# furcelay/gigalens

Hardware: AMD Instinct MI355X
Metric: forward+grad lens sims/sec, 128x128 px batch 1024; achieved HBM GB/s vs peak (higher is better)
Workload: dtype f32; 1 GPU; C2: EPL+shear lens, Sersic source, 128x128 px, batch 1024 per GPU, fp32 (BASELINE.json configs[1]); samples_per_gpu=1024, pixels=16384, z_dim=13, mode=fwdgrad, parallelism=single GPU

## Files before the change

### gigalens_amd/csrc/gigalens_hip.hip

```cpp
#include <algorithm>
#include <cmath>
#include <memory>
#include <cstdarg>
#include <cstdio>
#include <cstdlib>
#include <cstring>
#include <new>
#include <vector>

#include "gl_host_tables.h"
#include "gl_host.hip.h"
#include "gl_static.hip.h"
#include "gl_post.hip.h"
#include "gl_frontend.hip.h"
#include "gl_finalize.hip.h"

using namespace glk;

static thread_local char g_err[512] = "";

namespace glk {
int fail(int code, const char* fmt, ...) {
  va_list ap;
  va_start(ap, fmt);
  vsnprintf(g_err, sizeof(g_err), fmt, ap);
  va_end(ap);
  return code;
}
}

namespace {

int env_int(const char* name, int dflt) {
  const char* s = getenv(name);
  return (s && *s) ? atoi(s) : dflt;
}

void chunking(const gl_model* m, int B, int* chunk, int* n_chunks) {
  const long long tile_px = (long long)WG * 4;
  long long want = std::max<long long>((768 + B - 1) / B, ((long long)m->N + 8191) / 8192);
  if (m->target_wgs_set || !m->static_id) want = std::max<long long>(1, (m->target_wgs + B - 1) / B);
  long long per = ((long long)m->N + want - 1) / want;
  per = std::max(tile_px, (per + tile_px - 1) / tile_px * tile_px);
  if (m->chunk_px_override > 0) per = m->chunk_px_override;
  *chunk = (int)per;
  *n_chunks = (int)(((long long)m->N + per - 1) / per);
}

bool wave_front_end(const gl_model* m) { return m->has_epl && (int)m->comps.size() <= 64 && m->wave_prep; }
bool order_in_front_end(const gl_model* m, int B) {
  return wave_front_end(m) && m->use_order && m->order_fused && m->epl_comp >= 0 && B >= 2;
}

int tail_plan(const gl_model* m, int B, int n_chunks, int* tail_from, int* n_rows) {
  *tail_from = B;
  *n_rows = n_chunks;
  const bool pair_epl = m->pair && (m->static_id == ST_EPLSHEAR_SERSIC || m->static_id == ST_EPLSHEAR_SERSIC_SERSIC);
  if (m->tail_rows == 0 || !pair_epl || m->has_post || !order_in_front_end(m, B) || B > 1024) return 0;
  const int tiles = (m->N + 2 * WG - 1) / (2 * WG);
  const int slots = 256 * (m->static_id == ST_EPLSHEAR_SERSIC ? 3 : 2);
  int n_tail = m->tail_n, rows = m->tail_rows;
  if (n_tail < 0) {
    const long long wgs = (long long)B * n_chunks, rem = wgs % slots;
    if (wgs < slots || rem * 4 < slots) return 0;
    n_tail = (int)(rem / n_chunks);
  }
  if (rows < 0) rows = 2 * n_chunks;
  if (n_tail <= 0 || n_tail > B || rows > tiles || rows == n_chunks) return 0;
  *tail_from = B - n_tail;
  *n_rows = std::max(n_chunks, rows);
  return rows;
}

PostArgs post_args(const gl_model* m, float scale) {
  PostArgs p{};
  p.keff = m->d_psf;
  p.KH = m->KH; p.KW = m->KW; p.pt = m->pad_t; p.pl = m->pad_l;
  p.Hs = m->height; p.Ws = m->width; p.ss = m->supersample;
  p.H = m->height / m->supersample; p.W = m->width / m->supersample;
  p.scale = scale;
  return p;
}
constexpr bool corr_reachable(int kwp, int ncj, int ox) { return !(ox == 16 && kwp > 28) && !(ncj == 2 && kwp > 20); }
template <int KWP, int ST, int KS, int NCJ, int OX>
bool corr_launch(dim3 grid, size_t sh, hipStream_t stream, const float* in, float* out, const CorrArgs& a, std::atomic<const void*>* last) {
  if constexpr (corr_reachable(KWP, NCJ, OX)) {
    auto* fn = gl_corr_pair_kernel<KWP, ST, KS, NCJ, OX>;
    if (sh > 64 * 1024) {
      static const hipError_t big = hipFuncSetAttribute(reinterpret_cast<const void*>(fn), hipFuncAttributeMaxDynamicSharedMemorySize, 80 * 1024);
      if (big != hipSuccess) return false;
    }
    hipLaunchKernelGGL(fn, grid, dim3(CORR_GT * KS), sh, stream, in, out, a);
    if (last) last->store(reinterpret_cast<const void*>(fn), std::memory_order_relaxed);
    return true;
  } else {
    return false;
  }
}
bool launch_corr(const gl_model::CorrPlan& pl, int B, const float* in, float* out, float scale, hipStream_t stream, int dbg = 0,
                 int max_pairs_env = 0, int corr_wide = 1, std::atomic<const void*>* last = nullptr) {
  if (!pl.ok) return false;
  CorrArgs a = pl.args;
  a.B = B;
  a.scale = scale;
  a.dbg = dbg;
  a.vec = (a.Wi % 4 == 0 && a.Wout % 4 == 0 && ((reinterpret_cast<uintptr_t>(in) | reinterpret_cast<uintptr_t>(out)) & 15) == 0) ? 1 : 0;
  const bool wide = pl.ST == 2 && a.ncj == 1 && pl.KWP <= 28 && pl.max_KH <= 28 && corr_wide;
  const int ox = wide ? 16 : CORR_OX, ks = wide ? 8 : pl.ST == 2 ? 4 : 2;
  const int TR = (CORR_TR - 1) * pl.ST + pl.max_KH, TC = corr_tile_width((CORR_TCG * ox - 1) * pl.ST + pl.KWP) | 1;
  const size_t sh = std::max((size_t)TR * TC * sizeof(float2), (size_t)(ks - 1) * a.ncj * ox * CORR_GT * sizeof(float2) +
                                                                   (size_t)2 * CORR_TR * CORR_TCG * ox * a.ncj * sizeof(float));
  if (sh > (wide ? 80 : 64) * 1024) return false;
  const int max_pairs = max_pairs_env > 0 ? max_pairs_env : 65535 / a.n_class;
  if ((B + 1) / 2 > max_pairs) {
    for (int b_lo = 0; b_lo < B; b_lo += 2 * max_pairs) {
      const int nb = std::min(B - b_lo, 2 * max_pairs);
      if (!launch_corr(pl, nb, in + (size_t)b_lo * a.Hi * a.Wi, out + (size_t)b_lo * a.Hout * a.Wout, scale, stream, dbg, max_pairs_env, corr_wide, last)) return false;
    }
    return true;
  }
  const dim3 grid((pl.max_Wo + CORR_TCG * ox - 1) / (CORR_TCG * ox), (pl.max_Ho + CORR_TR - 1) / CORR_TR,
                  (unsigned)(a.n_class * ((B + 1) / 2)));
#define GL_CORR(KWP_, ST_, KS_, NCJ_, OX_) return corr_launch<KWP_, ST_, KS_, NCJ_, OX_>(grid, sh, stream, in, out, a, last);
#define GL_CORR_W(ST_, KS_, NCJ_, OX_)                                                                                          \
  switch (pl.KWP) {                                                                                                             \
    case 4: GL_CORR(4, ST_, KS_, NCJ_, OX_) case 8: GL_CORR(8, ST_, KS_, NCJ_, OX_) case 12: GL_CORR(12, ST_, KS_, NCJ_, OX_)     \
    case 16: GL_CORR(16, ST_, KS_, NCJ_, OX_) case 20: GL_CORR(20, ST_, KS_, NCJ_, OX_) case 24: GL_CORR(24, ST_, KS_, NCJ_, OX_) \
    case 28: GL_CORR(28, ST_, KS_, NCJ_, OX_) case 32: GL_CORR(32, ST_, KS_, NCJ_, OX_)                                          \
    default: return false;                                                                                                      \
  }
  if (wide) { GL_CORR_W(2, 8, 1, 16) }
  if (pl.ST == 2 && a.ncj == 1) { GL_CORR_W(2, 4, 1, CORR_OX) }
  if (pl.ST == 1 && a.ncj == 1) { GL_CORR_W(1, 2, 1, CORR_OX) }
  if (pl.ST == 1 && a.ncj == 2) { GL_CORR_W(1, 2, 2, CORR_OX) }
#undef GL_CORR_W
#undef GL_CORR
  return false;
}

}

namespace glk {

LaunchPlan launch_plan(const gl_model* m, int B) {
  LaunchPlan p{};
  chunking(m, B, &p.chunk, &p.n_chunks);
  p.tail_rows = tail_plan(m, B, p.n_chunks, &p.tail_from, &p.n_rows);
  return p;
}

Workspace carve(const gl_model* m, int B, void* base, const LaunchPlan& plan) {
  Workspace w{};
  size_t off = 0;
  char* p = (char*)base;
  w.derived = (float*)(p + off);
  off += align_up((size_t)B * m->D * sizeof(float), 256);
  w.partial = (float*)(p + off);
  off += align_up((size_t)B * plan.n_rows * m->A * sizeof(float), 256);
  w.params = (float*)(p + off);
  off += align_up((size_t)B * std::max(m->P, 1) * sizeof(float), 256);
  w.order = (int*)(p + off);
  off += align_up((size_t)B * sizeof(int), 256);
  w.cost = (int*)(p + off);
  off += align_up((size_t)B * sizeof(int), 256);
  if (m->G) {
    w.gal_dyn = (float*)(p + off);
    off += align_up((size_t)B * m->G * GM_ND * sizeof(float), 256);
  }
  if (m->pos_J) {
    auto take = [&](size_t n) { float* q = (float*)(p + off); off += align_up(n * sizeof(float), 256); return q; };
    w.pos_w = take((size_t)B * m->pos_J * 6);
    w.pos_adj = take((size_t)B * m->pos_J * 3);
    w.pos_g = take((size_t)B * m->pos_J * std::max(m->P, 1));
    w.pos_fam = take((size_t)B * m->pos_F * 2);
    w.pos_ll = take(B);
    w.pos_chi2 = take(B);
    w.pos_grad = take((size_t)B * std::max(m->P, 1));
    w.pos_dadj = take((size_t)B * m->pos_J);
  }
  if (m->has_post) {
    w.img_ss = (float*)(p + off);
    off += align_up((size_t)B * m->height * m->width * sizeof(float), 256);
    w.img_tmp = (float*)(p + off);
    off += align_up((size_t)B * (m->height / m->supersample) * (m->width / m->supersample) * sizeof(float), 256);
    w.stats = (float*)(p + off);
    off += align_up((size_t)B * 2 * sizeof(float), 256);
  } else if (m->mp_K >= 2) {
    w.img_tmp = (float*)(p + off);
    off += align_up((size_t)B * m->height * m->width * sizeof(float), 256);
    w.stats = (float*)(p + off);
    off += align_up((size_t)B * 2 * sizeof(float), 256);
  }
  w.bytes = off;
  return w;
}

MainArgs base_args(const gl_model* m, const Workspace& w, int chunk) {
  MainArgs a{};
  a.comps = m->d_comps;
  a.n_lens = m->n_lens;
  a.n_ll = m->n_ll;
  a.n_src = m->n_src;
  a.derived = w.derived;
  a.D = m->D;
  a.A = m->A;
  a.Apad = m->Apad;
  a.ncols = m->ncols;
  a.gx = m->d_gx;
  a.gy = m->d_gy;
  a.pix = m->d_pix;
  a.N = m->N;
  a.chunk = chunk;
  a.img_stride = (long long)m->height * m->width;
  a.out_scale = m->conversion_factor;
  a.partial = w.partial;
  a.shp_tab = m->d_shp_tab;
  a.nfw_tab = m->d_nfw_tab;
  a.neutral = m->d_nfw_tab ? m->d_nfw_tab + 2 * glh::kNfwNodes : nullptr;
  a.grid_rmax = m->shp_cull ? m->grid_rmax : -1.f;
  a.dbg = m->dbg_flags;
  a.careful_tiles = m->careful_tiles;
  a.shp_stride = m->shp_stride;
  a.parts = 7u;
  a.cats = m->d_cats;
  a.gal_static = m->d_gal_static;
  a.gal_dyn = w.gal_dyn;
  a.G = m->G;
  a.scaled_first = m->cats.empty() ? -1 : m->cats[0].dev.comp;
  a.series = m->d_series;
  a.interp = m->d_interp;
  a.interp_mass = m->d_interp_mass;
  a.src_scale = m->src_scaled ? m->d_src_scale.get() : nullptr;
  return a;
}

int check_ready(const gl_model* m, bool with_series, bool counted) {
  const int no_cat = m->n_scaled - (int)m->cats.size(), no_field = m->n_series - m->n_series_set;
  if (no_cat)
    return counted ? fail(GL_EINVAL, "%d GL_SCALED component(s) without a catalogue (gl_model_set_catalogue)", no_cat)
                   : fail(GL_EINVAL, "GL_SCALED component without a catalogue");
  if (m->n_interp != m->n_interp_set)
    return fail(GL_EINVAL, "%d GL_INTERPOL component(s) without an image (gl_model_set_light_image)", m->n_interp - m->n_interp_set);
  if (m->n_interp_mass != m->n_interp_mass_set)
    return fail(GL_EINVAL, "%d GL_INTERPOL_MASS component(s) without deflection maps (gl_model_set_lens_maps)",
                m->n_interp_mass - m->n_interp_mass_set);
  if (with_series && no_field)
    return counted ? fail(GL_EINVAL, "%d GL_SERIES component(s) without a coefficient field (gl_model_set_series)", no_field)
                   : fail(GL_EINVAL, "GL_SERIES component without a coefficient field");
  return GL_OK;
}

int refuse_planes(const gl_model* m, const char* what) {
  if (m && m->mp_K >= 2)
    return fail(GL_EUNSUPPORTED, "%s does not serve a model with %d lens planes (gl_model_set_lens_planes): lens maps, renders, "
                                 "pixel statistics and their gradients through the gl_multiplane_* entries alone", what, m->mp_K);
  return GL_OK;
}

int check_call(const gl_model* m, const void* params, int B, void* ws, size_t ws_bytes, LaunchPlan* plan, Workspace* w) {
  if (!m) return fail(GL_EINVAL, "model is null");
  if (!params) return fail(GL_EINVAL, "params is null");
  if (B <= 0 || B > 65535) return fail(GL_EINVAL, "batch size %d outside [1, 65535]", B);
  if (int rc = check_ready(m, true, true)) return rc;
  if (!ws) return fail(GL_EINVAL, "workspace is null");
  *plan = launch_plan(m, B);
  *w = carve(m, B, ws, *plan);
  if (ws_bytes < w->bytes) return fail(GL_ENOMEM, "workspace too small: %zu < %zu bytes", ws_bytes, w->bytes);
  return GL_OK;
}

int check_scales(const float* scales, int n, int expect, const char* what, bool* any) {
  if (!scales) return fail(GL_EINVAL, "scales is null");
  if (n != expect) return fail(GL_EINVAL, "%d scales for %d %s", n, expect, what);
  *any = false;
  for (int i = 0; i < n; ++i) {
    if (!(std::isfinite(scales[i]) && scales[i] > 0.f)) return fail(GL_EINVAL, "scale %d (%g) is not finite and > 0", i, scales[i]);
    *any = *any || scales[i] != 1.f;
  }
  return GL_OK;
}

int run_prep(const gl_model* m, const float* params, const float* z, int B, const LaunchPlan& plan, const Workspace& w,
             hipStream_t stream) {
  const int n_comp = (int)m->comps.size(), d_z = z ? m->d_z : 0;
  const ZCol* zcols = z ? m->d_zcols.get() : nullptr;
  const int* src = z ? m->d_src.get() : nullptr;
  const float* const_row = z ? m->d_const.get() : nullptr;
  float* rows_out = z ? w.params : nullptr;
  int* cost = m->epl_comp >= 0 ? w.cost : nullptr;
  if (wave_front_end(m)) {
    const bool ord = order_in_front_end(m, B);
    const size_t row_bytes = (size_t)4 * m->P * sizeof(float), rows = (m->prep_lds && row_bytes <= 48 * 1024) ? row_bytes : 0;
    const int split_rank = plan.tail_rows ? plan.tail_from : -1;
    hipLaunchKernelGGL(gl_prep_wave_kernel, dim3((B + 3) / 4 + (ord ? 1 : 0)), dim3(256), rows, stream, m->d_comps.get(), n_comp,
                       params, z, d_z, zcols, src, const_row, m->P, B, rows_out, w.derived, m->D, cost, m->epl_comp,
                       ord ? w.order : nullptr, rows ? 1 : 0, split_rank, m->d_interp.get(), m->d_interp_mass.get());
  } else {
    hipLaunchKernelGGL(gl_prep_kernel, dim3((B * n_comp + 127) / 128), dim3(128), 0, stream, m->d_comps.get(), n_comp, params, z,
                       d_z, zcols, src, const_row, m->P, B, rows_out, w.derived, m->D, cost, m->epl_comp, m->d_interp.get(),
                       m->d_interp_mass.get());
  }
  if (m->G) {
    const long long total = (long long)B * m->G;
    hipLaunchKernelGGL(gl_galprep_kernel, dim3((unsigned)((total + 127) / 128)), dim3(128), 0, stream, m->d_comps, m->d_cats,
// ... 1163 lines not shown
```

### gigalens_amd/csrc/gl_kernels.hip.h

```cpp
#pragma once
#include <hip/hip_runtime.h>
#include "gl_profiles.h"
#include "gl_dpie.h"
#include "gl_extra.h"
#include "gl_interp.h"
#include "gl_interp_mass.h"
#include "gl_vec.hip.h"
#include "gl_members.hip.h"
#include "gl_series.h"
#include "gl_shapelets.hip.h"

namespace glk {
using namespace glp;

struct CompDesc {
  int kind, iparam;
  unsigned flags;
  int p_off;
  int d_off;
  int a_off;
  int n_acc;
  int n_par;
  int lin_off;
};

struct CatDev {
  int base_kind, n_gal;
  int g_off;
  int comp;
  int col[3];
  int pad;
};

struct SeriesDev {
  const float* coef;
  const float* hcoef;
  float r0;
  int order;
};

using InterpDev = InterpTab<float>;
using InterpMassDev = InterpMassTab<float>;

struct PointAt {
  long long pt;
  int b;
  float x, y;
  __device__ __forceinline__ PointAt(long long pt_, int b_, long long i, int xy_batched, const float* x_, const float* y_)
      : pt(pt_), b(b_), x(xy_batched ? x_[i] : x_[pt_]), y(xy_batched ? y_[i] : y_[pt_]) {}
  __device__ __forceinline__ PointAt(long long i, int B, int xy_batched, const float* x_, const float* y_)
      : PointAt(i / B, (int)(i - i / B * B), i, xy_batched, x_, y_) {}
};

struct ZCol {
  int param_col;
  int bijector;
  int prior;
  float a, b, lo, hi, log_norm;
};
struct FinArgs {
  int n_comp, P, A, d_z;
  const float* params;
  float *loglike, *chi2, *grad;
  const float* z;
  const ZCol* zcols;
  float *logprob, *grad_z;
  float chi2_scale;
  const float* extra_stats;
  int use_partial;
  const float *pos_ll, *pos_chi2, *pos_grad;
  float pos_chi2_scale;
  const CatDev* cats;
};

enum Mode : int { IMG_FWD = 0, IMG_BWD = 1, LL_FWD = 2, LL_GRAD = 3, IMG_BASIS = 4 };
constexpr int WG = 256;
constexpr int NSTAT = 4;

struct MainArgs {
  const CompDesc* comps;
  int n_lens, n_ll, n_src;
  const float* derived;
  int D, A, Apad, ncols;
  const float* gx;
  const float* gy;
  const int* pix;
  int N, chunk;
  float* img;
  const float* gimg;
  long long img_stride;
  float out_scale;
  const float* obs;
  const float* err;
  const float* mask;
  float bg2, inv_t;
  float* partial;
  const float* shp_tab;
  int shp_stride;
  const int* order;
  int tail_rows, tail_from, n_rows, n_samples;
  unsigned parts;
  const CatDev* cats;
  const float* gal_static;
  const float* gal_dyn;
  int G;
  int scaled_first;
  int n_lin;
  const SeriesDev* series;
  const float* nfw_tab;
  const float* src_scale;
  const InterpDev* interp;
  const InterpMassDev* interp_mass;
  const float* neutral;
  float grid_rmax;
  int blk_w;
  int careful_tiles;
  int dbg;
};

#ifdef GL_EXPERIMENTS
#define GL_DBG(flags, bit) (((flags) & (bit)) != 0)
#else
#define GL_DBG(flags, bit) false
#endif

__device__ __forceinline__ float dpp_add(float v, int ctrl, int row_mask) {
  int r;
  switch (ctrl) {
    case 0x111: r = __builtin_amdgcn_update_dpp(0, __builtin_bit_cast(int, v), 0x111, 0xF, 0xF, true); break;
    case 0x112: r = __builtin_amdgcn_update_dpp(0, __builtin_bit_cast(int, v), 0x112, 0xF, 0xF, true); break;
    case 0x114: r = __builtin_amdgcn_update_dpp(0, __builtin_bit_cast(int, v), 0x114, 0xF, 0xF, true); break;
    case 0x118: r = __builtin_amdgcn_update_dpp(0, __builtin_bit_cast(int, v), 0x118, 0xF, 0xF, true); break;
    case 0x142: r = __builtin_amdgcn_update_dpp(0, __builtin_bit_cast(int, v), 0x142, 0xA, 0xF, false); break;
    default: r = __builtin_amdgcn_update_dpp(0, __builtin_bit_cast(int, v), 0x143, 0xC, 0xF, false); break;
  }
  (void)row_mask;
  return v + __builtin_bit_cast(float, r);
}
__device__ __forceinline__ float wave_sum63(float v) {
  v = dpp_add(v, 0x111, 0xF);
  v = dpp_add(v, 0x112, 0xF);
  v = dpp_add(v, 0x114, 0xF);
  v = dpp_add(v, 0x118, 0xF);
  v = dpp_add(v, 0x142, 0xA);
  v = dpp_add(v, 0x143, 0xC);
  return v;
}
__device__ __forceinline__ float quad_sum(float v) {
  v += __builtin_bit_cast(float, __builtin_amdgcn_update_dpp(0, __builtin_bit_cast(int, v), 0xB1, 0xF, 0xF, true));
  v += __builtin_bit_cast(float, __builtin_amdgcn_update_dpp(0, __builtin_bit_cast(int, v), 0x4E, 0xF, 0xF, true));
  return v;
}
__device__ __forceinline__ float dpp_xor1(float v) {
  return __builtin_bit_cast(float, __builtin_amdgcn_update_dpp(0, __builtin_bit_cast(int, v), 0xB1, 0xF, 0xF, true));
}
__device__ __forceinline__ float dpp_xor2(float v) {
  return __builtin_bit_cast(float, __builtin_amdgcn_update_dpp(0, __builtin_bit_cast(int, v), 0x4E, 0xF, 0xF, true));
}
__device__ __forceinline__ float quad_transpose_sum(float v0, float v1, float v2, float v3, bool odd, bool hi) {
  const float r01 = (odd ? v1 : v0) + dpp_xor1(odd ? v0 : v1);
  const float r23 = (odd ? v3 : v2) + dpp_xor1(odd ? v2 : v3);
  return (hi ? r23 : r01) + dpp_xor2(hi ? r01 : r23);
}

__device__ __forceinline__ float row_sum15(float v) {
  v = dpp_add(v, 0x111, 0xF);
// ... 724 lines not shown
```

### gigalens_amd/csrc/gl_pair.hip.h

```cpp
#pragma once
#include "gl_static.hip.h"
#include "gl_vec.hip.h"

namespace glk {

#ifdef GL_HAVE_USER
template <class V, int CODE> __device__ __forceinline__ void user_mass_fwd_v(const float* d, V x, V y, V& bx, V& by) {
  constexpr unsigned body = (unsigned)user_code_body(CODE);
  if constexpr (sizeof(V) == sizeof(float)) {
    float ax, ay;
    glu::mass_fwd(body, d, x, y, ax, ay);
    bx -= ax; by -= ay;
  } else {
    float ax0, ay0, ax1, ay1;
    glu::mass_fwd(body, d, x.x, y.x, ax0, ay0);
    glu::mass_fwd(body, d, x.y, y.y, ax1, ay1);
    bx -= V{ax0, ax1};
    by -= V{ay0, ay1};
  }
}
template <class V, int CODE> __device__ __forceinline__ void user_mass_vjp_v(const float* d, V x, V y, V gx, V gy, V* acc) {
  constexpr unsigned body = (unsigned)user_code_body(CODE);
  constexpr int NPAR = user_code_npar(CODE);
  float t0[NPAR > 0 ? NPAR : 1], t1[NPAR > 0 ? NPAR : 1];
#pragma unroll
  for (int k = 0; k < NPAR; ++k) { t0[k] = 0.f; t1[k] = 0.f; }
  if constexpr (sizeof(V) == sizeof(float)) {
    glu::mass_vjp(body, d, x, y, gx, gy, t0);
#pragma unroll
    for (int k = 0; k < NPAR; ++k) acc[k] += t0[k];
  } else {
    glu::mass_vjp(body, d, x.x, y.x, gx.x, gy.x, t0);
    glu::mass_vjp(body, d, x.y, y.y, gx.y, gy.y, t1);
#pragma unroll
    for (int k = 0; k < NPAR; ++k) acc[k] += V{t0[k], t1[k]};
  }
}
template <class V, int CODE> __device__ __forceinline__ V user_light_fwd_v(const float* d, V x, V y) {
  constexpr unsigned body = (unsigned)user_code_body(CODE);
  if constexpr (sizeof(V) == sizeof(float)) return glu::light_fwd(body, d, x, y);
  else return V{glu::light_fwd(body, d, x.x, y.x), glu::light_fwd(body, d, x.y, y.y)};
}
template <class V, int CODE, bool SRC>
__device__ __forceinline__ void user_light_vjp_v(const float* d, V x, V y, V g, V* acc, V& gpx, V& gpy) {
  constexpr unsigned body = (unsigned)user_code_body(CODE);
  constexpr int NPAR = user_code_npar(CODE);
  float t0[NPAR > 0 ? NPAR : 1], t1[NPAR > 0 ? NPAR : 1];
#pragma unroll
  for (int k = 0; k < NPAR; ++k) { t0[k] = 0.f; t1[k] = 0.f; }
  if constexpr (sizeof(V) == sizeof(float)) {
    float dgx = 0.f, dgy = 0.f;
    glu::light_vjp(body, d, x, y, g, t0, dgx, dgy);
#pragma unroll
    for (int k = 0; k < NPAR; ++k) acc[k] += t0[k];
    if (SRC) { gpx += dgx; gpy += dgy; }
  } else {
    float dgx0 = 0.f, dgy0 = 0.f, dgx1 = 0.f, dgy1 = 0.f;
    glu::light_vjp(body, d, x.x, y.x, g.x, t0, dgx0, dgy0);
    glu::light_vjp(body, d, x.y, y.y, g.y, t1, dgx1, dgy1);
#pragma unroll
    for (int k = 0; k < NPAR; ++k) acc[k] += V{t0[k], t1[k]};
    if (SRC) { gpx += V{dgx0, dgx1}; gpy += V{dgy0, dgy1}; }
  }
}
#endif

template <int MODE, class V, int WAVES, class LK, class LLK, class SK>
__global__ void __launch_bounds__(WG, WAVES) gl_pair_kernel(MainArgs a) {
  constexpr int NL = LK::n, NLL = LLK::n, NS = SK::n, NLIGHT = NLL + NS;
  constexpr bool GRAD = (MODE == IMG_BWD || MODE == LL_GRAD);
  constexpr int W = sizeof(V) / sizeof(float);
  extern __shared__ float smem[];
  float* s_d = smem;
  float* s_acc = smem + ((a.D + 3) & ~3);
  const int tid = threadIdx.x;
  int rank = blockIdx.y, row = blockIdx.x, n_rows = gridDim.x, my_rows = gridDim.x;
  int p0 = row * a.chunk, p1 = min(p0 + a.chunk, a.N);
  if (a.tail_rows > 0) {
    n_rows = a.n_rows;
    if (rank >= a.tail_from) {
      const int j = (rank - a.tail_from) * (int)gridDim.x + row;
      rank = a.tail_from + j / a.tail_rows;
      if (rank >= a.n_samples) return;
      row = j % a.tail_rows;
      my_rows = a.tail_rows;
      const int tiles = (a.N + W * WG - 1) / (W * WG);
      p0 = (int)((long long)row * tiles / a.tail_rows) * (W * WG);
      p1 = min((int)((long long)(row + 1) * tiles / a.tail_rows) * (W * WG), a.N);
    }
  }
  const int b = a.order ? a.order[rank] : rank;
  const CompDesc* __restrict__ comps = a.comps;
  const float* __restrict__ gder = a.derived + (size_t)b * a.D;
  if (!GL_DBG(a.dbg, 4)) {
    if (a.D <= WG) {
      if (tid < a.D) s_d[tid] = gder[tid];
    } else {
      for (int i = tid; i < a.D; i += WG) s_d[i] = gder[i];
    }
  }
  __syncthreads();
  constexpr int NACC_L = [] { int n = 0; for (int i = 0; i < NL; ++i) n += static_nacc(LK::kinds[i]); return n; }();
  constexpr int NACC_C = [] {
    int n = 0;
    for (int i = 0; i < NLL; ++i) n += static_nacc(LLK::kinds[i]);
    for (int i = 0; i < NS; ++i) n += static_nacc(SK::kinds[i]);
    return n;
  }();
  V accL[NACC_L > 0 ? NACC_L : 1];
  V accC[NACC_C > 0 ? NACC_C : 1];
#pragma unroll
  for (int k = 0; k < NACC_L; ++k) accL[k] = V(0.f);
#pragma unroll
  for (int k = 0; k < NACC_C; ++k) accC[k] = V(0.f);
  V st0 = V(0.f), st1 = V(0.f);
  V wsum = V(0.f);
  int n_whole = 0;
  const float* dL[NL > 0 ? NL : 1];
  const float* dC[NLIGHT > 0 ? NLIGHT : 1];
#pragma unroll
  for (int i = 0; i < NL; ++i) dL[i] = s_d + comps[i].d_off;
#pragma unroll
  for (int i = 0; i < NLIGHT; ++i) dC[i] = s_d + comps[NL + i].d_off;
  const bool has_err = a.err != nullptr, has_mask = a.mask != nullptr, has_pix = a.pix != nullptr;
  auto plane = [](const float* p) { return __builtin_amdgcn_make_buffer_rsrc(const_cast<float*>(p), (short)0, -1, 0x00020000); };
  const auto r_obs = plane(a.obs), r_err = plane(a.err);

  auto tile = [&](int base, auto check_tag, auto err_tag) -> bool {
    constexpr bool CHECK = decltype(check_tag)::value;
    constexpr bool FAST = !CHECK;
    unsigned worst = 0;
    constexpr int ERR = decltype(err_tag)::value;
    const bool herr = ERR == 2 ? has_err : ERR == 1;
    unsigned jj[W], pidx[W];
    bool valid[W];
    V x, y, vmask = V(1.f);
#pragma unroll
    for (int w = 0; w < W; ++w) {
      int j = base + w * WG + tid;
      valid[w] = CHECK ? (j < p1) : true;
      jj[w] = (unsigned)(valid[w] ? j : p1 - 1);
      pidx[w] = (CHECK && has_pix) ? (unsigned)a.pix[jj[w]] : jj[w];
    }
    unsigned jo[W], po[W];
#pragma unroll
    for (int w = 0; w < W; ++w) { jo[w] = jj[w] << 2; po[w] = pidx[w] << 2; }
    auto ldf = [](const float* base, unsigned byte_off) { return *reinterpret_cast<const float*>(reinterpret_cast<const char*>(base) + byte_off); };
    auto ldb = [](auto rsrc, const float* base, unsigned byte_off) {
      if constexpr (CHECK) return *reinterpret_cast<const float*>(reinterpret_cast<const char*>(base) + byte_off);
      else return __uint_as_float(__builtin_amdgcn_raw_buffer_load_b32(rsrc, byte_off, 0, 0));
    };
    if constexpr (W == 2) {
      x = V{ldf(a.gx, jo[0]), ldf(a.gx, jo[1])};
      y = V{ldf(a.gy, jo[0]), ldf(a.gy, jo[1])};
      if (CHECK) vmask = V{valid[0] ? 1.f : 0.f, valid[1] ? 1.f : 0.f};
    } else {
      x = ldf(a.gx, jo[0]);
      y = ldf(a.gy, jo[0]);
      if (CHECK) vmask = valid[0] ? 1.f : 0.f;
    }
    V bx = x, by = y, m = V(0.f);
    EplStateV<V> est[NL > 0 ? NL : 1];
    SieStateV<V> sie_st[NL > 0 ? NL : 1];
    SerStateV<V> sst[NLIGHT > 0 ? NLIGHT : 1];
    static_for([&](auto I) {
      constexpr int i = decltype(I)::value;
      constexpr int kind = LK::kinds[i];
      if constexpr (kind == K_EPL) epl_fwd_v<V, GRAD, const float*, FAST>(dL[i], gder + comps[i].d_off, x, y, bx, by, est[i], &worst);
      else if constexpr (kind == K_SIE) sie_fwd_v<V>(dL[i], x, y, bx, by, (FAST && GRAD) ? &sie_st[i] : nullptr);
      else if constexpr (kind == K_SHEAR) shear_fwd_v<V>(dL[i], x, y, bx, by);
#ifdef GL_HAVE_USER
      else if constexpr (is_user_code(kind)) user_mass_fwd_v<V, kind>(dL[i], x, y, bx, by);
#endif
      else sis_fwd_v<V, FAST>(dL[i], x, y, bx, by, &worst);
    }, std::make_integer_sequence<int, NL>{});
    static_for([&](auto I) {
      constexpr int i = decltype(I)::value;
      constexpr bool src = i >= NLL;
      constexpr int lkind = src ? SK::kinds[src ? i - NLL : 0] : LLK::kinds[src ? 0 : i];
      constexpr bool ell = lkind != K_SERSIC;
#ifdef GL_HAVE_USER
      if constexpr (is_user_code(lkind)) m += user_light_fwd_v<V, lkind>(dC[i], src ? bx : x, src ? by : y);
      else
#endif
      m += sersic_fwd_v<V, ell, FAST>(dC[i], src ? bx : x, src ? by : y, sst[i], GRAD ? &worst : nullptr);
    }, std::make_integer_sequence<int, NLIGHT>{});
    auto nanp = m != m;
    if constexpr (FAST) {
      if ((__builtin_amdgcn_ballot_w64(worst > kGuardWidth) | __builtin_amdgcn_ballot_w64(any_nan(m))) != 0) return false;
      m = m * a.out_scale;
    } else {
      m = (nanp ? V(0.f) : m) * a.out_scale;
    }
    if (MODE == IMG_FWD) {
      float* row = a.img + (size_t)b * a.img_stride;
      if constexpr (W == 2) {
        if (valid[0]) row[pidx[0]] = m.x;
        if (valid[1]) row[pidx[1]] = m.y;
      } else {
        if (valid[0]) row[pidx[0]] = m;
      }
      return true;
    }
    V gm;
    if (MODE == IMG_BWD) {
      const float* row = a.gimg + (size_t)b * a.img_stride;
      V g;
      if constexpr (W == 2) g = V{row[pidx[0]], row[pidx[1]]}; else g = row[pidx[0]];
      gm = FAST ? g * a.out_scale : (nanp ? V(0.f) : (CHECK ? g * vmask : g) * a.out_scale);
    } else {
      V o, w = vmask, e = V(1.f);
      if constexpr (W == 2) {
        o = V{ldb(r_obs, a.obs, po[0]), ldb(r_obs, a.obs, po[1])};
        if (CHECK && has_mask) w = w * V{ldf(a.mask, po[0]), ldf(a.mask, po[1])};
        if (herr) e = V{ldb(r_err, a.err, po[0]), ldb(r_err, a.err, po[1])};
      } else {
        o = ldb(r_obs, a.obs, po[0]);
        if (CHECK && has_mask) w = w * ldf(a.mask, po[0]);
        if (herr) e = ldb(r_err, a.err, po[0]);
      }
      V dmo = m - o;
      V s2 = herr ? e * e : m * a.inv_t + a.bg2;
      V is2 = rcp(s2);
      V nm = log2_(s2);
      V c2 = __builtin_elementwise_fma(nm, V(0.f), dmo * dmo * is2);
      if (CHECK) {
        auto use = w != V(0.f);
        st0 += use ? c2 * w : V(0.f);
        st1 += use ? nm * w : V(0.f);
        wsum += w;
      } else {
        st0 += c2;
        st1 += nm;
      }
      if (MODE == LL_GRAD) {
        V g = herr ? -(dmo * is2) : (dmo * dmo * is2 - 1.f) * (is2 * (0.5f * a.inv_t)) - dmo * is2;
        gm = FAST ? g * a.out_scale : (nanp ? V(0.f) : (CHECK ? g * w : g) * a.out_scale);
      }
    }
    if constexpr (GRAD) {
      V gbx = V(0.f), gby = V(0.f);
      static_for([&](auto I) {
        constexpr int i = decltype(I)::value;
        constexpr bool src = i >= NLL;
        constexpr int off = [] {
          int n = 0;
          for (int j = 0; j < i; ++j) n += static_nacc(j < NLL ? LLK::kinds[j < NLL ? j : 0] : SK::kinds[j >= NLL ? j - NLL : 0]);
          return n;
        }();
        constexpr int lkind = src ? SK::kinds[src ? i - NLL : 0] : LLK::kinds[src ? 0 : i];
        constexpr bool ell = lkind != K_SERSIC;
#ifdef GL_HAVE_USER
        if constexpr (is_user_code(lkind)) user_light_vjp_v<V, lkind, src>(dC[i], src ? bx : x, src ? by : y, gm, accC + off, gbx, gby);
        else
#endif
        sersic_vjp_v<V, src, ell, FAST>(dC[i], sst[i], gm, accC + off, gbx, gby);
      }, std::make_integer_sequence<int, NLIGHT>{});
      gbx = -gbx;
      gby = -gby;
      static_for([&](auto I) {
        constexpr int i = decltype(I)::value;
        constexpr int kind = LK::kinds[i];
        constexpr int off = [] { int n = 0; for (int j = 0; j < i; ++j) n += static_nacc(LK::kinds[j]); return n; }();
        if constexpr (kind == K_EPL) epl_vjp_v<V>(dL[i], gbx, gby, est[i], accL + off);
        else if constexpr (kind == K_SIE) sie_vjp_v<V>(dL[i], x, y, gbx, gby, accL + off, FAST ? &sie_st[i] : nullptr);
        else if constexpr (kind == K_SHEAR) shear_vjp_v<V>(x, y, gbx, gby, accL + off);
#ifdef GL_HAVE_USER
        else if constexpr (is_user_code(kind)) user_mass_vjp_v<V, kind>(dL[i], x, y, gbx, gby, accL + off);
#endif
        else sis_vjp_v<V, FAST>(dL[i], x, y, gbx, gby, accL + off);
      }, std::make_integer_sequence<int, NL>{});
    }
    return true;
  };
  {
    bool sample_ok = !a.careful_tiles;
    static_for([&](auto I) {
      constexpr int i = decltype(I)::value;
      constexpr int lkind = i < NLL ? LLK::kinds[i < NLL ? i : 0] : SK::kinds[i >= NLL ? i - NLL : 0];
      if constexpr (!is_user_code(lkind)) sample_ok = sample_ok && sersic_fast_ok(gder + comps[NL + i].d_off);
    }, std::make_integer_sequence<int, NLIGHT>{});
    const bool plain = !has_mask && !has_pix && sample_ok;
    int base = p0;
    if (GL_DBG(a.dbg, 1)) base = p1;
    if (plain) {
      if (has_err) {
        for (; base + WG * W <= p1; base += WG * W, ++n_whole)
          if (!tile(base, std::false_type{}, std::integral_constant<int, 1>{})) break;
      } else {
        for (; base + WG * W <= p1; base += WG * W, ++n_whole)
          if (!tile(base, std::false_type{}, std::integral_constant<int, 0>{})) break;
      }
    }
    for (; base < p1; base += WG * W) tile(base, std::true_type{}, std::integral_constant<int, 2>{});
  }
  if (MODE == IMG_FWD) return;
  auto norm_term = [](float l2sum, float w) { return (l2sum + w * 2.6514961294723187f) * (float)kLn2; };
  float* out = a.partial + ((size_t)b * n_rows + row) * a.A;
  if (row == 0)
    for (int i = my_rows * a.A + tid; i < n_rows * a.A; i += WG) out[i] = 0.f;
  if (!GRAD) {
    for (int i = tid; i < 4 * a.Apad; i += WG) s_acc[i] = 0.f;
    __syncthreads();
  }
  if constexpr (GRAD) {
    constexpr int NV = NSTAT + NACC_L + NACC_C, NVP = (NV + 3) & ~3;
    float vals[NVP];
#pragma unroll
    for (int k = 0; k < NVP; ++k) vals[k] = 0.f;
    vals[0] = (MODE == LL_GRAD) ? hsum(st0) : 0.f;
    vals[1] = (MODE == LL_GRAD) ? norm_term(hsum(st1), hsum(wsum) + (float)(W * n_whole)) : 0.f;
    static_for([&](auto I) {
      constexpr int i = decltype(I)::value;
      constexpr int kind = LK::kinds[i];
      constexpr int off = [] { int n = 0; for (int j = 0; j < i; ++j) n += static_nacc(LK::kinds[j]); return n; }();
      constexpr int G = static_nacc(kind);
      float tmp[G];
#pragma unroll
      for (int k = 0; k < G; ++k) tmp[k] = hsum(accL[off + k]);
      if constexpr (kind == K_EPL) {
        tmp[EPLA_B] = tmp[EPLA_P0] * (dL[i][EPL_TM1] * dL[i][EPL_INVB]);
        tmp[EPLA_P0] *= rcp(dL[i][EPL_P0]);
        const float gxr = tmp[EPLA_CX], gyr = tmp[EPLA_CY], cc = dL[i][EPL_C], ss = dL[i][EPL_S];
        tmp[EPLA_CX] = -(gxr * cc - gyr * ss);
        tmp[EPLA_CY] = -(gxr * ss + gyr * cc);
      }
#pragma unroll
      for (int k = 0; k < G; ++k) vals[NSTAT + off + k] = tmp[k];
    }, std::make_integer_sequence<int, NL>{});
    static_for([&](auto I) {
      constexpr int i = decltype(I)::value;
      constexpr int off = [] {
        int n = 0;
        for (int j = 0; j < i; ++j) n += static_nacc(j < NLL ? LLK::kinds[j < NLL ? j : 0] : SK::kinds[j >= NLL ? j - NLL : 0]);
        return n;
      }();
      constexpr int lkind = i < NLL ? LLK::kinds[i < NLL ? i : 0] : SK::kinds[i >= NLL ? i - NLL : 0];
      if constexpr (is_user_code(lkind)) {
#pragma unroll
        for (int k = 0; k < static_nacc(lkind); ++k) vals[NSTAT + NACC_L + off + k] = hsum(accC[off + k]);
      } else {
#pragma unroll
        for (int k = 0; k < SER_NACC; ++k) vals[NSTAT + NACC_L + off + k] = hsum(accC[off + k]) * (k == SERA_INVN ? (float)kLn2 : 1.f);
      }
    }, std::make_integer_sequence<int, NLIGHT>{});
    const bool odd = tid & 1, hi = tid & 2;
    float* s_row16 = s_acc + (tid >> 4) * a.Apad;
#pragma unroll
    for (int g = 0; g < NVP / 4; ++g) {
      float r = quad_transpose_sum(vals[4 * g], vals[4 * g + 1], vals[4 * g + 2], vals[4 * g + 3], odd, hi);
      r = dpp_add(r, 0x114, 0xF);
      r = dpp_add(r, 0x118, 0xF);
      if ((tid & 15) >= 12 && 4 * g + (tid & 3) < NV) s_row16[4 * g + (tid & 3)] = r;
    }
    __syncthreads();
    for (int k = tid; k < NV; k += WG) {
      float v = 0.f;
#pragma unroll
      for (int j = 0; j < 16; ++j) v += s_acc[j * a.Apad + k];
      out[k] = v;
    }
    return;
  }
  float* s_row = s_acc + (tid >> 6) * a.Apad;
// ... 16 lines not shown
```

### gigalens_amd/csrc/gl_vec.hip.h

```cpp
#pragma once
#include <hip/hip_runtime.h>

#include "gl_profiles.h"

namespace glk {
using namespace glp;

typedef float v2f __attribute__((ext_vector_type(2)));

using glm::rcp;
using glm::sqrt_;
using glm::exp2_;
using glm::log2_;
using glm::atan_;
using glm::atanh_;

__device__ __forceinline__ v2f rcp(v2f a) { return v2f{glm::rcp(a.x), glm::rcp(a.y)}; }
__device__ __forceinline__ v2f sqrt_(v2f a) { return v2f{glm::sqrt_(a.x), glm::sqrt_(a.y)}; }
__device__ __forceinline__ float rsq_(float a) { return __builtin_amdgcn_rsqf(a); }
__device__ __forceinline__ v2f rsq_(v2f a) { return v2f{__builtin_amdgcn_rsqf(a.x), __builtin_amdgcn_rsqf(a.y)}; }
__device__ __forceinline__ v2f exp2_(v2f a) { return v2f{glm::exp2_(a.x), glm::exp2_(a.y)}; }
__device__ __forceinline__ v2f log2_(v2f a) { return v2f{glm::log2_(a.x), glm::log2_(a.y)}; }
__device__ __forceinline__ v2f atan_(v2f a) { return v2f{glm::atan_(a.x), glm::atan_(a.y)}; }
__device__ __forceinline__ v2f atanh_(v2f a) { return v2f{glm::atanh_(a.x), glm::atanh_(a.y)}; }
template <class V> __device__ __forceinline__ V vexp(V x) {
  const float hi = (float)kLog2e;
  const float lo = (float)(kLog2e - (double)(float)kLog2e);
  V t = x * hi;
  V e = __builtin_elementwise_fma(x, V(hi), -t) + x * lo;
  V p = exp2_(t);
  return __builtin_elementwise_fma(p, e * (float)kLn2, p);
}
template <> __device__ __forceinline__ float vexp<float>(float x) { return glm::exp_(x); }
template <class V> __device__ __forceinline__ V vlog(V x) { return log2_(x) * (float)kLn2; }
__device__ __forceinline__ float floor_at(float a, float lo) { return __builtin_fmaxf(a, lo); }
__device__ __forceinline__ v2f floor_at(v2f a, float lo) { return v2f{__builtin_fmaxf(a.x, lo), __builtin_fmaxf(a.y, lo)}; }
__device__ __forceinline__ float clamp3(float a, float lo, float hi) { return __builtin_amdgcn_fmed3f(a, lo, hi); }
__device__ __forceinline__ v2f clamp3(v2f a, float lo, float hi) { return v2f{__builtin_amdgcn_fmed3f(a.x, lo, hi), __builtin_amdgcn_fmed3f(a.y, lo, hi)}; }
template <class V> __device__ __forceinline__ V vmin(V a, V b) { return a < b ? a : b; }
template <class V> __device__ __forceinline__ V vmax(V a, V b) { return a > b ? a : b; }
__device__ __forceinline__ float hsum(float a) { return a; }
__device__ __forceinline__ float hsum(v2f a) { return a.x + a.y; }

constexpr unsigned kGuardWidth = __builtin_bit_cast(unsigned, 1e10f) - __builtin_bit_cast(unsigned, 1e-10f);
constexpr float kGuardRadLo = 1e-15f;
__device__ __forceinline__ void guard_range(unsigned& worst, float v, float lo) {
  worst = max(worst, __float_as_uint(v) - __builtin_bit_cast(unsigned, lo));
}
__device__ __forceinline__ void guard_range(unsigned& worst, v2f v, float lo) {
  const float v0 = v.x, v1 = v.y;
  worst = max(max(worst, __float_as_uint(v0) - __builtin_bit_cast(unsigned, lo)), __float_as_uint(v1) - __builtin_bit_cast(unsigned, lo));
}
__device__ __forceinline__ bool any_nan(float a) { return a != a; }
__device__ __forceinline__ bool any_nan(v2f a) { return __builtin_isunordered(a.x, a.y); }

template <class V> struct EplStateV {
  V xr, yr, inv, invc, L2, P, Cs, Ss, arx, ary;
  V f0, f1, t0, t1;
};

typedef const float __attribute__((address_space(4)))* gptr4;
typedef float vf4 __attribute__((ext_vector_type(4)));
template <class T, class P> struct gl_rebind;
template <class T> struct gl_rebind<T, const float*> { using type = const T*; };
template <class T> struct gl_rebind<T, gptr4> { using type = const T __attribute__((address_space(4)))*; };

template <class V, bool GRAD, class P = const float*, bool FAST = false>
__device__ __forceinline__ void epl_fwd_v(const float* d, const P gd, V x, V y, V& bx, V& by,
                                          EplStateV<V>& st, unsigned* worst = nullptr) {
  using PInt = typename gl_rebind<int, P>::type;
  using PRow = typename gl_rebind<vf4, P>::type;
  const float c = d[EPL_C], s = d[EPL_S], q = d[EPL_Q];
  V dx = x - d[EPL_CX], dy = y - d[EPL_CY];
  st.xr = dx * c + dy * s;
  st.yr = dy * c - dx * s;
  V X = st.xr * q;
  V r2 = X * X + st.yr * st.yr;
  V r = rsq_(r2);
  V iRc;
  if constexpr (FAST) {
    guard_range(*worst, r, 1e-10f);
    st.inv = r;
    st.Cs = X * r;
    iRc = r;
    st.invc = r;
  } else {
    auto pos = r2 > V(0.f);
    st.inv = pos ? r : V(0.f);
    st.Cs = pos ? X * r : V(1.f);
    iRc = clamp3(r, 1e-10f, 1e10f);
    st.invc = (iRc == r) ? r : V(0.f);
  }
  st.Ss = st.yr * st.inv;
  V twoc = (st.Cs * st.Cs - st.Ss * st.Ss) * 2.f;
  const int K = ((PInt)gd)[EPL_KI];
  const PRow gtab = (PRow)(gd + EPL_TAB);
  V o1, o2, f1 = V(0.f), f2 = V(0.f), t1 = V(0.f), t2 = V(0.f);
  auto term = [&](const vf4 ck, V& b1, V& b2, V& g1, V& g2, V& h1, V& h2) {
    b2 = __builtin_elementwise_fma(twoc, b1, V(ck.x)) - b2;
    if (GRAD) {
      g2 = __builtin_elementwise_fma(twoc, g1, V(ck.z)) - g2;
      h2 = __builtin_elementwise_fma(twoc, h1, V(ck.w)) - h2;
    }
  };
  auto four = [&](const vf4 r0, const vf4 r1, const vf4 r2, const vf4 r3) {
    term(r3, o1, o2, f1, f2, t1, t2);
    term(r2, o2, o1, f2, f1, t2, t1);
    term(r1, o1, o2, f1, f2, t1, t2);
    term(r0, o2, o1, f2, f1, t2, t1);
  };
  auto four_first = [&](const vf4 r0, const vf4 r1, const vf4 r2, const vf4 r3) {
    o1 = __builtin_elementwise_fma(twoc, V(r3.x), V(r2.x));
    o2 = __builtin_elementwise_fma(twoc, o1, V(r1.x)) - V(r3.x);
    o1 = __builtin_elementwise_fma(twoc, o2, V(r0.x)) - o1;
    if (GRAD) {
      f1 = __builtin_elementwise_fma(twoc, V(r3.z), V(r2.z));
      f2 = __builtin_elementwise_fma(twoc, f1, V(r1.z)) - V(r3.z);
      f1 = __builtin_elementwise_fma(twoc, f2, V(r0.z)) - f1;
      t1 = __builtin_elementwise_fma(twoc, V(r3.w), V(r2.w));
      t2 = __builtin_elementwise_fma(twoc, t1, V(r1.w)) - V(r3.w);
      t1 = __builtin_elementwise_fma(twoc, t2, V(r0.w)) - t1;
    }
  };
  int trips = (K + 4) >> 2;
  int row = 4 * trips - 4;
  PRow p = gtab + row;
  vf4 a0 = p[0], a1 = p[1], a2 = p[2], a3 = p[3];
  row = row >= 4 ? row - 4 : 0;
  p = gtab + row;
  vf4 b0 = p[0], b1 = p[1], b2 = p[2], b3 = p[3];
  four_first(a0, a1, a2, a3);
  if (--trips != 0) {
    while (true) {
      row = row >= 4 ? row - 4 : 0;
      p = gtab + row;
      a0 = p[0]; a1 = p[1]; a2 = p[2]; a3 = p[3];
      four(b0, b1, b2, b3);
      if (--trips == 0) break;
      row = row >= 4 ? row - 4 : 0;
      p = gtab + row;
      b0 = p[0]; b1 = p[1]; b2 = p[2]; b3 = p[3];
      four(a0, a1, a2, a3);
      if (--trips == 0) break;
    }
  }
  const V o0 = o1, ob = o2;
  if (GRAD) { st.f0 = f1; st.f1 = f2; st.t0 = t1; st.t1 = t2; }
  const V Ox = (o0 - ob) * st.Cs, Oy = (o0 + ob) * st.Ss;
  st.L2 = log2_(iRc * d[EPL_B]);
  st.P = exp2_(st.L2 * d[EPL_TM1]) * d[EPL_P0];
  const V arx = st.P * Ox, ary = st.P * Oy;
  st.arx = arx;
  st.ary = ary;
  bx -= arx * c - ary * s;
  by -= arx * s + ary * c;
}

template <class V>
__device__ __forceinline__ void epl_vjp_v(const float* d, V gx, V gy, const EplStateV<V>& st, V* acc) {
  const float c = d[EPL_C], s = d[EPL_S], q = d[EPL_Q], tm1 = d[EPL_TM1];
  const V P = st.P, arx = st.arx, ary = st.ary;
  V grx = gx * c + gy * s, gry = gy * c - gx * s;
  V g_phi = gry * arx - grx * ary;
  const V cross = g_phi;
  V gW_W = grx * arx + gry * ary;
  V gOx = P * grx, gOy = P * gry;
  V A = gOx * st.Cs, B = gOy * st.Ss, C = gOy * st.Cs, D = gOx * st.Ss;
  V dotp = A + B, dotm = B - A, crsm = C - D, crsp = C + D;
  V g_ang = cross + (st.f0 * crsm - st.f1 * crsp) * d[EPL_F2];
  V g_t = st.t0 * dotp + st.t1 * dotm;
  V g_f = st.f0 * dotp + st.f1 * dotm;
  g_t += gW_W * (st.L2 * (float)kLn2);
  V gR0 = -(gW_W * st.invc) * tm1;
  V gai = g_ang * st.inv;
  V gX = gR0 * st.Cs - gai * st.Ss;
  V gyr = gR0 * st.Ss + gai * st.Cs;
  V gxr = gX * q;
  g_phi += gxr * st.yr - gyr * st.xr;
  acc[EPLA_CX] += gxr;
  acc[EPLA_CY] += gyr;
  acc[EPLA_PHI] += g_phi;
  acc[EPLA_Q] += gX * st.xr;
  acc[EPLA_T] += g_t;
  acc[EPLA_F] += g_f;
  acc[EPLA_P0] += gW_W;
}

template <class V> struct SieStateV { V xr, yr, ipsi, u, v, fu, fv; };
template <class V> __device__ __forceinline__ SieStateV<V> sie_state_v(const float* d, V x, V y) {
  const float c = d[SIE_C], s = d[SIE_S], q = d[SIE_Q], sq = d[SIE_SQ];
  V dx = x - d[SIE_CX], dy = y - d[SIE_CY];
  SieStateV<V> st;
  st.xr = dx * c + dy * s;
  st.yr = dy * c - dx * s;
  st.ipsi = rcp(sqrt_(st.xr * st.xr * (q * q) + st.yr * st.yr));
  st.u = st.xr * st.ipsi * sq;
  st.v = st.yr * st.ipsi * sq;
  st.fu = atan_(st.u);
  st.fv = atanh_(st.v);
  return st;
}
template <class V> __device__ __forceinline__ void sie_fwd_v(const float* d, V x, V y, V& bx, V& by, SieStateV<V>* keep = nullptr) {
  const float c = d[SIE_C], s = d[SIE_S], A = d[SIE_A];
  const SieStateV<V> st = sie_state_v<V>(d, x, y);
  V arx = st.fu * A, ary = st.fv * A;
  bx -= arx * c - ary * s;
  by -= arx * s + ary * c;
  if (keep) *keep = st;
}
template <class V> __device__ __forceinline__ void sie_vjp_v(const float* d, V x, V y, V gx, V gy, V* acc, const SieStateV<V>* kept = nullptr) {
// ... 183 lines not shown
```

Measured before the change: 12.57 million sims/s.

## Hoist per-sample loads ahead of barrier and pass component offsets in kernel args

Moves component derived-data offsets into the kernel argument struct so they no longer come from a global CompDesc load. Issues the staging load, the Sersic fast-check loads and the first EPL table trip before the shared-memory barrier, and prefetches observed/error pixels early in fast likelihood modes. Tail-row index math switches to unsigned arithmetic, guarded by new overflow checks on the host. The intent is to hide global-load latency behind setup work, at the cost of more live registers, which may lower occupancy.

```diff
diff --git a/gigalens_amd/csrc/gigalens_hip.hip b/gigalens_amd/csrc/gigalens_hip.hip
--- a/gigalens_amd/csrc/gigalens_hip.hip
+++ b/gigalens_amd/csrc/gigalens_hip.hip
@@ -67,6 +67,7 @@
   }
   if (rows < 0) rows = 2 * n_chunks;
   if (n_tail <= 0 || n_tail > B || rows > tiles || rows == n_chunks) return 0;
+  if ((long long)rows * tiles > 0x7fffffffLL || (long long)n_tail * rows + n_chunks > 0x7fffffffLL) return 0;
   *tail_from = B - n_tail;
   *n_rows = std::max(n_chunks, rows);
   return rows;
@@ -220,6 +221,7 @@
   a.grid_rmax = m->shp_cull ? m->grid_rmax : -1.f;
   a.dbg = m->dbg_flags;
   a.careful_tiles = m->careful_tiles;
+  for (int i = 0; i < kPairComps && i < (int)m->comps.size(); ++i) a.d_off[i] = m->comps[i].d_off;
   a.shp_stride = m->shp_stride;
   a.parts = 7u;
   a.cats = m->d_cats;
diff --git a/gigalens_amd/csrc/gl_kernels.hip.h b/gigalens_amd/csrc/gl_kernels.hip.h
--- a/gigalens_amd/csrc/gl_kernels.hip.h
+++ b/gigalens_amd/csrc/gl_kernels.hip.h
@@ -76,12 +76,14 @@
 enum Mode : int { IMG_FWD = 0, IMG_BWD = 1, LL_FWD = 2, LL_GRAD = 3, IMG_BASIS = 4 };
 constexpr int WG = 256;
 constexpr int NSTAT = 4;
+constexpr int kPairComps = 12;
 
 struct MainArgs {
   const CompDesc* comps;
   int n_lens, n_ll, n_src;
   const float* derived;
   int D, A, Apad, ncols;
+  int d_off[kPairComps];
   const float* gx;
   const float* gy;
   const int* pix;
diff --git a/gigalens_amd/csrc/gl_pair.hip.h b/gigalens_amd/csrc/gl_pair.hip.h
--- a/gigalens_amd/csrc/gl_pair.hip.h
+++ b/gigalens_amd/csrc/gl_pair.hip.h
@@ -70,6 +70,7 @@
   constexpr int NL = LK::n, NLL = LLK::n, NS = SK::n, NLIGHT = NLL + NS;
   constexpr bool GRAD = (MODE == IMG_BWD || MODE == LL_GRAD);
   constexpr int W = sizeof(V) / sizeof(float);
+  static_assert(NL + NLIGHT <= kPairComps, "MainArgs::d_off holds the first kPairComps components");
   extern __shared__ float smem[];
   float* s_d = smem;
   float* s_acc = smem + ((a.D + 3) & ~3);
@@ -79,25 +80,35 @@
   if (a.tail_rows > 0) {
     n_rows = a.n_rows;
     if (rank >= a.tail_from) {
-      const int j = (rank - a.tail_from) * (int)gridDim.x + row;
-      rank = a.tail_from + j / a.tail_rows;
+      const unsigned j = (unsigned)((rank - a.tail_from) * (int)gridDim.x + row), rows = (unsigned)a.tail_rows;
+      const unsigned s = j / rows;
+      rank = a.tail_from + (int)s;
       if (rank >= a.n_samples) return;
-      row = j % a.tail_rows;
+      row = (int)(j - s * rows);
       my_rows = a.tail_rows;
-      const int tiles = (a.N + W * WG - 1) / (W * WG);
-      p0 = (int)((long long)row * tiles / a.tail_rows) * (W * WG);
-      p1 = min((int)((long long)(row + 1) * tiles / a.tail_rows) * (W * WG), a.N);
+      const unsigned tiles = (unsigned)((a.N + W * WG - 1) / (W * WG));
+      p0 = (int)((unsigned)row * tiles / rows) * (W * WG);
+      p1 = min((int)((unsigned)(row + 1) * tiles / rows) * (W * WG), a.N);
     }
   }
   const int b = a.order ? a.order[rank] : rank;
-  const CompDesc* __restrict__ comps = a.comps;
   const float* __restrict__ gder = a.derived + (size_t)b * a.D;
+  const int i_stage = min(tid, a.D - 1);
+  const float staged = gder[i_stage];
+  bool sample_ok = !a.careful_tiles;
+  static_for([&](auto I) {
+    constexpr int i = decltype(I)::value;
+    constexpr int lkind = i < NLL ? LLK::kinds[i < NLL ? i : 0] : SK::kinds[i >= NLL ? i - NLL : 0];
+    if constexpr (!is_user_code(lkind)) sample_ok = sample_ok & sersic_fast_ok(gder + a.d_off[NL + i]);
+  }, std::make_integer_sequence<int, NLIGHT>{});
+  EplFirstTrip first[NL > 0 ? NL : 1];
+  static_for([&](auto I) {
+    constexpr int i = decltype(I)::value;
+    if constexpr (LK::kinds[i] == K_EPL) first[i] = epl_first_trip(gder + a.d_off[i]);
+  }, std::make_integer_sequence<int, NL>{});
   if (!GL_DBG(a.dbg, 4)) {
-    if (a.D <= WG) {
-      if (tid < a.D) s_d[tid] = gder[tid];
-    } else {
-      for (int i = tid; i < a.D; i += WG) s_d[i] = gder[i];
-    }
+    s_d[i_stage] = staged;
+    for (int i = tid + WG; i < a.D; i += WG) s_d[i] = gder[i];
   }
   __syncthreads();
   constexpr int NACC_L = [] { int n = 0; for (int i = 0; i < NL; ++i) n += static_nacc(LK::kinds[i]); return n; }();
@@ -119,9 +130,9 @@
   const float* dL[NL > 0 ? NL : 1];
   const float* dC[NLIGHT > 0 ? NLIGHT : 1];
 #pragma unroll
-  for (int i = 0; i < NL; ++i) dL[i] = s_d + comps[i].d_off;
-#pragma unroll
-  for (int i = 0; i < NLIGHT; ++i) dC[i] = s_d + comps[NL + i].d_off;
+  for (int i = 0; i < NL; ++i) dL[i] = s_d + a.d_off[i];
+#pragma unroll
+  for (int i = 0; i < NLIGHT; ++i) dC[i] = s_d + a.d_off[NL + i];
   const bool has_err = a.err != nullptr, has_mask = a.mask != nullptr, has_pix = a.pix != nullptr;
   auto plane = [](const float* p) { return __builtin_amdgcn_make_buffer_rsrc(const_cast<float*>(p), (short)0, -1, 0x00020000); };
   const auto r_obs = plane(a.obs), r_err = plane(a.err);
@@ -159,6 +170,17 @@
       y = ldf(a.gy, jo[0]);
       if (CHECK) vmask = valid[0] ? 1.f : 0.f;
     }
+    constexpr bool EARLY = FAST && (MODE == LL_FWD || MODE == LL_GRAD);
+    V o_early = V(0.f), e_early = V(1.f);
+    if constexpr (EARLY) {
+      if constexpr (W == 2) {
+        o_early = V{ldb(r_obs, a.obs, jo[0]), ldb(r_obs, a.obs, jo[1])};
+        if (herr) e_early = V{ldb(r_err, a.err, jo[0]), ldb(r_err, a.err, jo[1])};
+      } else {
+        o_early = ldb(r_obs, a.obs, jo[0]);
+        if (herr) e_early = ldb(r_err, a.err, jo[0]);
+      }
+    }
     V bx = x, by = y, m = V(0.f);
     EplStateV<V> est[NL > 0 ? NL : 1];
     SieStateV<V> sie_st[NL > 0 ? NL : 1];
@@ -166,7 +188,7 @@
     static_for([&](auto I) {
       constexpr int i = decltype(I)::value;
       constexpr int kind = LK::kinds[i];
-      if constexpr (kind == K_EPL) epl_fwd_v<V, GRAD, const float*, FAST>(dL[i], gder + comps[i].d_off, x, y, bx, by, est[i], &worst);
+      if constexpr (kind == K_EPL) epl_fwd_v<V, GRAD, const float*, FAST>(dL[i], gder + a.d_off[i], x, y, bx, by, est[i], &worst, &first[i]);
       else if constexpr (kind == K_SIE) sie_fwd_v<V>(dL[i], x, y, bx, by, (FAST && GRAD) ? &sie_st[i] : nullptr);
       else if constexpr (kind == K_SHEAR) shear_fwd_v<V>(dL[i], x, y, bx, by);
 #ifdef GL_HAVE_USER
@@ -188,10 +210,11 @@
     auto nanp = m != m;
     if constexpr (FAST) {
       if ((__builtin_amdgcn_ballot_w64(worst > kGuardWidth) | __builtin_amdgcn_ballot_w64(any_nan(m))) != 0) return false;
-      m = m * a.out_scale;
     } else {
-      m = (nanp ? V(0.f) : m) * a.out_scale;
-    }
+      m = nanp ? V(0.f) : m;
+    }
+    const V m_raw = m;
+    m = m * a.out_scale;
     if (MODE == IMG_FWD) {
       float* row = a.img + (size_t)b * a.img_stride;
       if constexpr (W == 2) {
@@ -210,7 +233,10 @@
       gm = FAST ? g * a.out_scale : (nanp ? V(0.f) : (CHECK ? g * vmask : g) * a.out_scale);
     } else {
       V o, w = vmask, e = V(1.f);
-      if constexpr (W == 2) {
+      if constexpr (EARLY) {
+        o = o_early;
+        e = e_early;
+      } else if constexpr (W == 2) {
         o = V{ldb(r_obs, a.obs, po[0]), ldb(r_obs, a.obs, po[1])};
         if (CHECK && has_mask) w = w * V{ldf(a.mask, po[0]), ldf(a.mask, po[1])};
         if (herr) e = V{ldb(r_err, a.err, po[0]), ldb(r_err, a.err, po[1])};
@@ -219,7 +245,7 @@
         if (CHECK && has_mask) w = w * ldf(a.mask, po[0]);
         if (herr) e = ldb(r_err, a.err, po[0]);
       }
-      V dmo = m - o;
+      V dmo = __builtin_elementwise_fma(m_raw, V(a.out_scale), -o);
       V s2 = herr ? e * e : m * a.inv_t + a.bg2;
       V is2 = rcp(s2);
       V nm = log2_(s2);
@@ -274,12 +300,6 @@
     return true;
   };
   {
-    bool sample_ok = !a.careful_tiles;
-    static_for([&](auto I) {
-      constexpr int i = decltype(I)::value;
-      constexpr int lkind = i < NLL ? LLK::kinds[i < NLL ? i : 0] : SK::kinds[i >= NLL ? i - NLL : 0];
-      if constexpr (!is_user_code(lkind)) sample_ok = sample_ok && sersic_fast_ok(gder + comps[NL + i].d_off);
-    }, std::make_integer_sequence<int, NLIGHT>{});
     const bool plain = !has_mask && !has_pix && sample_ok;
     int base = p0;
     if (GL_DBG(a.dbg, 1)) base = p1;
diff --git a/gigalens_amd/csrc/gl_vec.hip.h b/gigalens_amd/csrc/gl_vec.hip.h
--- a/gigalens_amd/csrc/gl_vec.hip.h
+++ b/gigalens_amd/csrc/gl_vec.hip.h
@@ -65,9 +65,20 @@
 template <class T> struct gl_rebind<T, const float*> { using type = const T*; };
 template <class T> struct gl_rebind<T, gptr4> { using type = const T __attribute__((address_space(4)))*; };
 
+struct EplFirstTrip { int K; vf4 r0, r1, r2, r3; };
+template <class P> __device__ __forceinline__ EplFirstTrip epl_first_trip(const P gd) {
+  using PInt = typename gl_rebind<int, P>::type;
+  using PRow = typename gl_rebind<vf4, P>::type;
+  EplFirstTrip f;
+  f.K = ((PInt)gd)[EPL_KI];
+  const PRow p = (PRow)(gd + EPL_TAB) + (4 * ((f.K + 4) >> 2) - 4);
+  f.r0 = p[0]; f.r1 = p[1]; f.r2 = p[2]; f.r3 = p[3];
+  return f;
+}
+
 template <class V, bool GRAD, class P = const float*, bool FAST = false>
 __device__ __forceinline__ void epl_fwd_v(const float* d, const P gd, V x, V y, V& bx, V& by,
-                                          EplStateV<V>& st, unsigned* worst = nullptr) {
+                                          EplStateV<V>& st, unsigned* worst = nullptr, const EplFirstTrip* first = nullptr) {
   using PInt = typename gl_rebind<int, P>::type;
   using PRow = typename gl_rebind<vf4, P>::type;
   const float c = d[EPL_C], s = d[EPL_S], q = d[EPL_Q];
@@ -93,7 +104,7 @@
   }
   st.Ss = st.yr * st.inv;
   V twoc = (st.Cs * st.Cs - st.Ss * st.Ss) * 2.f;
-  const int K = ((PInt)gd)[EPL_KI];
+  const int K = first ? first->K : ((PInt)gd)[EPL_KI];
   const PRow gtab = (PRow)(gd + EPL_TAB);
   V o1, o2, f1 = V(0.f), f2 = V(0.f), t1 = V(0.f), t2 = V(0.f);
   auto term = [&](const vf4 ck, V& b1, V& b2, V& g1, V& g2, V& h1, V& h2) {
@@ -125,7 +136,9 @@
   int trips = (K + 4) >> 2;
   int row = 4 * trips - 4;
   PRow p = gtab + row;
-  vf4 a0 = p[0], a1 = p[1], a2 = p[2], a3 = p[3];
+  vf4 a0, a1, a2, a3;
+  if (first) { a0 = first->r0; a1 = first->r1; a2 = first->r2; a3 = first->r3; }
+  else { a0 = p[0]; a1 = p[1]; a2 = p[2]; a3 = p[3]; }
   row = row >= 4 ? row - 4 : 0;
   p = gtab + row;
   vf4 b0 = p[0], b1 = p[1], b2 = p[2], b3 = p[3];
```

Result: no change. 12.69 million sims/s, median of 6 (+0.9%).
